# crockwell/rel_pose

Hardware: AMD Instinct MI355X
Metric: image-pairs/sec fwd+bwd @384x384, 1/2/4/8 MI355X; R,t err vs ref (higher is better)
Workload: dtype f32; 1 GPU; train.py step (ViTEss fwd + geodesic loss + bwd + grad all-reduce + clip + Adam), synthetic 384x384 pairs; scope=full, pairs_per_gpu=64, global_batch_pairs=64, parallelism=dp1, finite=True, gemm_operand_precision=exact fp32 MFMA, launch=eager

## Files before the change

__graft_entry__.py:

```python
import os
import subprocess
import sys

ROOT = os.path.dirname(os.path.abspath(__file__))
if ROOT not in sys.path:
    sys.path.insert(0, ROOT)


def build():
    import torch
    from rel_pose_amd import _build
    force = os.environ.get("RP_FORCE_BUILD", "" if torch.cuda.is_available() else "1") == "1"
    _build.build(force=force, verbose=True)
    from rel_pose_amd import _lib
    lib = _lib.load()
    assert lib.rp_abi_version() == _lib.ABI_VERSION and lib.rp_target_arch() == b"gfx950"
    assert lib.rp_abi_export_count() == _lib.ABI_EXPORTS == len(_lib.EXPORTS)
    assert _lib.load_readout().rp_readout_abi_version() == _lib.READOUT_ABI_VERSION
    assert _lib.load_eightpoint().rp_eightpoint_abi_version() == _lib.EIGHTPOINT_ABI_VERSION
    assert _lib.load_refine().rp_refine_abi_version() == _lib.REFINE_ABI_VERSION
    assert _lib.load_consensus().rp_consensus_abi_version() == _lib.CONSENSUS_ABI_VERSION
    assert _lib.load_submatch().rp_submatch_abi_version() == _lib.SUBMATCH_ABI_VERSION
    assert _lib.load_fivepoint().rp_fivepoint_abi_version() == _lib.FIVEPOINT_ABI_VERSION
    assert _lib.load_homography().rp_homography_abi_version() == _lib.HOMOGRAPHY_ABI_VERSION
    assert _lib.load_triangulate().rp_triangulate_abi_version() == _lib.TRIANGULATE_ABI_VERSION
    assert _lib.load_conv5x5().rp_conv5x5_abi_version() == _lib.CONV5X5_ABI_VERSION
    assert _lib.load_guided().rp_guided_abi_version() == _lib.GUIDED_ABI_VERSION
    assert _lib.load_rotation().rp_rotation_abi_version() == _lib.ROTATION_ABI_VERSION
    assert _lib.load_select().rp_select_abi_version() == _lib.SELECT_ABI_VERSION
    assert _lib.load_covariance().rp_covariance_abi_version() == _lib.COVARIANCE_ABI_VERSION
    assert _lib.load_resection().rp_resection_abi_version() == _lib.RESECTION_ABI_VERSION
    import rel_pose_amd.model
    import oracle.relpose_oracle
    print("build ok:", _lib.lib_path(), _build.READOUT_LIB, _build.EIGHTPOINT_LIB, _build.REFINE_LIB, _build.CONSENSUS_LIB, _build.SUBMATCH_LIB,
          _build.FIVEPOINT_LIB, _build.HOMOGRAPHY_LIB, _build.TRIANGULATE_LIB, _build.CONV5X5_LIB, _build.GUIDED_LIB, _build.ROTATION_LIB, _build.SELECT_LIB,
          _build.COVARIANCE_LIB, _build.RESECTION_LIB)


def smoke():
    import types

    import torch

    from oracle import relpose_oracle as O
    from rel_pose_amd import _lib
    from rel_pose_amd.model import ViTEss
    assert torch.cuda.is_available(), "smoke() needs cuda:0"
    _lib.load()
    torch.cuda.set_device(0)
    args = types.SimpleNamespace(noess="", pool_size=60, fc_hidden_size=512, fusion_transformer=True,
                                 transformer_depth=6, cross_features=False, use_single_softmax=False,
                                 no_pos_encoding=False, l1_pos_encoding=False)
    shapes = dict(O.vit_param_shapes())
    shapes.update(O.cnn_param_shapes())
    sd32, sd64 = O.make_state(shapes, torch.float32), O.make_state(shapes, torch.float64)
    model = ViTEss(args)
    model.load_state_dict(sd32)
    model = model.cuda().train()
    tok = O.synthetic_tokens(2)
    Gs = torch.tensor([0, 0, 0, 0, 0, 0, 1.0]).repeat(1, 2, 1)
    intr = torch.tensor([[30.0, 26.0, 12.0, 11.0]]).repeat(1, 2, 1)
    fmap = tok.permute(0, 2, 1).contiguous().view(2, 192, 24, 24).cuda().requires_grad_(True)
    out = model.forward_tokens(fmap, Gs.cuda(), intr.cuda())
    out[:, 1].square().sum().backward()
    t64 = tok.double().requires_grad_(True)
    ref = O.vit_ess_from_tokens(sd64, t64, Gs.double(), intr.double())
    ref[:, 1].square().sum().backward()
    t_err, q_err, ang = O.pose_errors(out.detach().cpu(), ref.detach())
    g_err = O.rel_err(fmap.grad.view(2, 192, 576).permute(0, 2, 1).cpu(), t64.grad)
    print("smoke: t_err=%.2e q_err=%.2e angle=%.2e rad, token-grad rel err=%.2e" % (t_err, q_err, ang, g_err))
    assert max(t_err, q_err) < 1e-4 and g_err < 2e-5
    print("smoke ok (HIP path vs CPU oracle)")


if __name__ == "__main__":
    build()
    if len(sys.argv) > 1 and sys.argv[1] == "smoke":
        smoke()
```

rel_pose_amd/_build.py:

```python
import os
import subprocess
import sys

HERE = os.path.dirname(os.path.abspath(__file__))
CSRC = os.path.join(HERE, "csrc")
LIB = os.path.join(HERE, "librelpose_hip.so")
SOURCES = ["gemm.hip", "gemm_dma.hip", "rowwise.hip", "attention.hip", "attention_bf16.hip", "dw192_bf16.hip", "dw192_f32.hip", "dw192_split3.hip", "dx_lnbwd_bf16.hip", "emm.hip", "emm_bf16.hip", "batchnorm.hip", "se3loss.hip", "geom.hip", "augment.hip", "mlp_fused.hip", "linear_rows.hip", "conv_stem.hip", "conv_stem_bf16.hip", "conv_stem_wgrad_bf16.hip", "conv_stem_wgrad_f32.hip", "conv3x3_bf16.hip", "conv3x3_wgrad_bf16.hip", "conv3x3_wgrad_f32.hip", "conv3x3_f32.hip", "conv3x3_c128_f32.hip"]
READOUT_CSRC = os.path.join(HERE, "csrc_readout")
READOUT_LIB = os.path.join(HERE, "librelpose_readout.so")
READOUT_SOURCES = ["emm_readout.hip"]
EIGHTPOINT_CSRC = os.path.join(HERE, "csrc_eightpoint")
EIGHTPOINT_LIB = os.path.join(HERE, "librelpose_eightpoint.so")
EIGHTPOINT_SOURCES = ["eight_point.hip"]
REFINE_CSRC = os.path.join(HERE, "csrc_refine")
REFINE_LIB = os.path.join(HERE, "librelpose_refine.so")
REFINE_SOURCES = ["refine_pose.hip"]
CONSENSUS_CSRC = os.path.join(HERE, "csrc_consensus")
CONSENSUS_LIB = os.path.join(HERE, "librelpose_consensus.so")
CONSENSUS_SOURCES = ["consensus.hip"]
SUBMATCH_CSRC = os.path.join(HERE, "csrc_submatch")
SUBMATCH_LIB = os.path.join(HERE, "librelpose_submatch.so")
SUBMATCH_SOURCES = ["submatch.hip"]
FIVEPOINT_CSRC = os.path.join(HERE, "csrc_fivepoint")
FIVEPOINT_LIB = os.path.join(HERE, "librelpose_fivepoint.so")
FIVEPOINT_SOURCES = ["five_point.hip"]
HOMOGRAPHY_CSRC = os.path.join(HERE, "csrc_homography")
HOMOGRAPHY_LIB = os.path.join(HERE, "librelpose_homography.so")
HOMOGRAPHY_SOURCES = ["homography.hip"]
TRIANGULATE_CSRC = os.path.join(HERE, "csrc_triangulate")
TRIANGULATE_LIB = os.path.join(HERE, "librelpose_triangulate.so")
TRIANGULATE_SOURCES = ["triangulate.hip"]
CONV5X5_CSRC = os.path.join(HERE, "csrc_conv5x5")
CONV5X5_LIB = os.path.join(HERE, "librelpose_conv5x5.so")
CONV5X5_SOURCES = ["conv5x5_dgrad_f32.hip"]
GUIDED_CSRC = os.path.join(HERE, "csrc_guided")
GUIDED_LIB = os.path.join(HERE, "librelpose_guided.so")
GUIDED_SOURCES = ["emm_guided.hip"]
ROTATION_CSRC = os.path.join(HERE, "csrc_rotation")
ROTATION_LIB = os.path.join(HERE, "librelpose_rotation.so")
ROTATION_SOURCES = ["rotation.hip"]
SELECT_CSRC = os.path.join(HERE, "csrc_select")
SELECT_LIB = os.path.join(HERE, "librelpose_select.so")
SELECT_SOURCES = ["select.hip"]
COVARIANCE_CSRC = os.path.join(HERE, "csrc_covariance")
COVARIANCE_LIB = os.path.join(HERE, "librelpose_covariance.so")
COVARIANCE_SOURCES = ["covariance.hip"]
RESECTION_CSRC = os.path.join(HERE, "csrc_resection")
RESECTION_LIB = os.path.join(HERE, "librelpose_resection.so")
RESECTION_SOURCES = ["resection.hip"]
ARCH = "gfx950"


def _hipcc():
    for c in (os.environ.get("HIPCC"), "/opt/rocm/bin/hipcc"):
        if c and os.path.exists(c):
            return c
    return "hipcc"


def _stale(lib, csrc, sources, headers):
    if not os.path.exists(lib):
        return True
    t = os.path.getmtime(lib)
    return any(os.path.getmtime(d) > t for d in [os.path.join(csrc, s) for s in sources] + headers)


def needs_build():
    return _stale(LIB, CSRC, SOURCES, _headers())


def readout_needs_build():
    return _stale(READOUT_LIB, READOUT_CSRC, READOUT_SOURCES, _readout_headers())


def eightpoint_needs_build():
    return _stale(EIGHTPOINT_LIB, EIGHTPOINT_CSRC, EIGHTPOINT_SOURCES, _eightpoint_headers())


def refine_needs_build():
    return _stale(REFINE_LIB, REFINE_CSRC, REFINE_SOURCES, _refine_headers())


def consensus_needs_build():
    return _stale(CONSENSUS_LIB, CONSENSUS_CSRC, CONSENSUS_SOURCES, _consensus_headers())


def submatch_needs_build():
    return _stale(SUBMATCH_LIB, SUBMATCH_CSRC, SUBMATCH_SOURCES, _submatch_headers())


def fivepoint_needs_build():
    return _stale(FIVEPOINT_LIB, FIVEPOINT_CSRC, FIVEPOINT_SOURCES, _fivepoint_headers())


def homography_needs_build():
    return _stale(HOMOGRAPHY_LIB, HOMOGRAPHY_CSRC, HOMOGRAPHY_SOURCES, _homography_headers())


def triangulate_needs_build():
    return _stale(TRIANGULATE_LIB, TRIANGULATE_CSRC, TRIANGULATE_SOURCES, _triangulate_headers())


def conv5x5_needs_build():
    return _stale(CONV5X5_LIB, CONV5X5_CSRC, CONV5X5_SOURCES, _conv5x5_headers())


def guided_needs_build():
    return _stale(GUIDED_LIB, GUIDED_CSRC, GUIDED_SOURCES, _guided_headers())


def rotation_needs_build():
    return _stale(ROTATION_LIB, ROTATION_CSRC, ROTATION_SOURCES, _rotation_headers())


def select_needs_build():
    return _stale(SELECT_LIB, SELECT_CSRC, SELECT_SOURCES, _select_headers())


def covariance_needs_build():
    return _stale(COVARIANCE_LIB, COVARIANCE_CSRC, COVARIANCE_SOURCES, _covariance_headers())


def resection_needs_build():
    return _stale(RESECTION_LIB, RESECTION_CSRC, RESECTION_SOURCES, _resection_headers())


def build(force=False, verbose=True):
    import fcntl
    with open(os.path.join(HERE, ".build.lock"), "w") as lock:
        fcntl.flock(lock, fcntl.LOCK_EX)
        try:
            if force or needs_build():
                _build_locked(verbose, force, LIB, CSRC, SOURCES, _headers())
            if force or readout_needs_build():
                _build_locked(verbose, force, READOUT_LIB, READOUT_CSRC, READOUT_SOURCES, _readout_headers())
            if force or eightpoint_needs_build():
                _build_locked(verbose, force, EIGHTPOINT_LIB, EIGHTPOINT_CSRC, EIGHTPOINT_SOURCES, _eightpoint_headers())
            if force or refine_needs_build():
                _build_locked(verbose, force, REFINE_LIB, REFINE_CSRC, REFINE_SOURCES, _refine_headers())
            if force or consensus_needs_build():
                _build_locked(verbose, force, CONSENSUS_LIB, CONSENSUS_CSRC, CONSENSUS_SOURCES, _consensus_headers())
            if force or submatch_needs_build():
                _build_locked(verbose, force, SUBMATCH_LIB, SUBMATCH_CSRC, SUBMATCH_SOURCES, _submatch_headers())
            if force or fivepoint_needs_build():
                _build_locked(verbose, force, FIVEPOINT_LIB, FIVEPOINT_CSRC, FIVEPOINT_SOURCES, _fivepoint_headers())
            if force or homography_needs_build():
                _build_locked(verbose, force, HOMOGRAPHY_LIB, HOMOGRAPHY_CSRC, HOMOGRAPHY_SOURCES, _homography_headers())
            if force or triangulate_needs_build():
                _build_locked(verbose, force, TRIANGULATE_LIB, TRIANGULATE_CSRC, TRIANGULATE_SOURCES, _triangulate_headers())
            if force or conv5x5_needs_build():
                _build_locked(verbose, force, CONV5X5_LIB, CONV5X5_CSRC, CONV5X5_SOURCES, _conv5x5_headers())
            if force or guided_needs_build():
                _build_locked(verbose, force, GUIDED_LIB, GUIDED_CSRC, GUIDED_SOURCES, _guided_headers())
            if force or rotation_needs_build():
                _build_locked(verbose, force, ROTATION_LIB, ROTATION_CSRC, ROTATION_SOURCES, _rotation_headers())
            if force or select_needs_build():
                _build_locked(verbose, force, SELECT_LIB, SELECT_CSRC, SELECT_SOURCES, _select_headers())
            if force or covariance_needs_build():
                _build_locked(verbose, force, COVARIANCE_LIB, COVARIANCE_CSRC, COVARIANCE_SOURCES, _covariance_headers())
            if force or resection_needs_build():
                _build_locked(verbose, force, RESECTION_LIB, RESECTION_CSRC, RESECTION_SOURCES, _resection_headers())
            return LIB
        finally:
            fcntl.flock(lock, fcntl.LOCK_UN)


def _headers():
    return [os.path.join(CSRC, h) for h in sorted(os.listdir(CSRC)) if h.endswith(".h")] + \
           [os.path.join(os.path.dirname(HERE), "include", "relpose_hip.h")]


def _readout_headers():
    return _headers() + [os.path.join(os.path.dirname(HERE), "include", "relpose_readout.h")]


def _eightpoint_headers():
    return _headers() + [os.path.join(os.path.dirname(HERE), "include", "relpose_eightpoint.h")]


def _refine_headers():
    return _headers() + [os.path.join(os.path.dirname(HERE), "include", "relpose_refine.h")]


def _consensus_headers():
    return _headers() + [os.path.join(os.path.dirname(HERE), "include", "relpose_consensus.h")]


def _submatch_headers():
    return _headers() + [os.path.join(os.path.dirname(HERE), "include", "relpose_submatch.h")]


def _fivepoint_headers():
    return _headers() + [os.path.join(os.path.dirname(HERE), "include", "relpose_fivepoint.h")]


def _homography_headers():
    return _headers() + [os.path.join(os.path.dirname(HERE), "include", "relpose_homography.h")]


def _triangulate_headers():
    return _headers() + [os.path.join(os.path.dirname(HERE), "include", "relpose_triangulate.h")]


def _conv5x5_headers():
    return _headers() + [os.path.join(os.path.dirname(HERE), "include", "relpose_conv5x5.h")]


def _guided_headers():
    return _headers() + [os.path.join(os.path.dirname(HERE), "include", "relpose_guided.h")]


def _rotation_headers():
    return _headers() + [os.path.join(os.path.dirname(HERE), "include", "relpose_rotation.h")]


def _select_headers():
    return _headers() + [os.path.join(os.path.dirname(HERE), "include", "relpose_select.h")]


def _covariance_headers():
    return _headers() + [os.path.join(COVARIANCE_CSRC, "sym5.h"), os.path.join(os.path.dirname(HERE), "include", "relpose_covariance.h")]


def _resection_headers():
    return _headers() + [os.path.join(os.path.dirname(HERE), "include", "relpose_resection.h")]


def _build_locked(verbose, force, lib, csrc, sources, headers):
    cc = _hipcc()
    objs = []
    procs = []
    hdr_t = max(os.path.getmtime(h) for h in headers)
    for s in sources:
        o = os.path.join(csrc, s.replace(".hip", ".o"))
        objs.append(o)
        if not force and os.path.exists(o) and os.path.getmtime(o) > max(hdr_t, os.path.getmtime(os.path.join(csrc, s))):
            continue
        cmd = [cc, "--offload-arch=" + ARCH, "-O3", "-std=c++17", "-fPIC", "-c", os.path.join(csrc, s), "-o", o]
        if verbose:
            print(" ".join(cmd), flush=True)
        procs.append((s, subprocess.Popen(cmd, stdout=subprocess.PIPE, stderr=subprocess.STDOUT)))
    for s, p in procs:
        out, _ = p.communicate()
        if p.returncode != 0:
            sys.stderr.write(out.decode())
            raise RuntimeError("hipcc failed on " + s)
    tmp = lib + ".tmp.%d" % os.getpid()
    cmd = [cc, "--offload-arch=" + ARCH, "-shared", "-fPIC", "-o", tmp] + objs
    if verbose:
        print(" ".join(cmd), flush=True)
    subprocess.check_call(cmd)
    os.replace(tmp, lib)
    return lib


if __name__ == "__main__":
    build(force="--force" in sys.argv)
```

rel_pose_amd/_lib.py:

```python
import ctypes
import keyword
import os
import re
from ctypes import POINTER, Structure, c_char_p, c_float, c_int, c_longlong, c_size_t, c_void_p

import torch

from . import _build

_LIB = None
HEADER = os.path.join(os.path.dirname(os.path.dirname(os.path.abspath(__file__))), "include", "relpose_hip.h")

_SCALARS = {"int": c_int, "float": c_float, "long long": c_longlong, "size_t": c_size_t}
_POINTEES = ("void", "float", "double", "int", "unsigned char")
_DEFINE = re.compile(r"#\s*define\s+(RP_\w+)\s+(-?\d+|\(-?\d+\))")
_DECL = re.compile(r"(const\s+)?(unsigned\s+char|long\s+long|\w+)\s*(\*?)\s*([A-Za-z_]\w*(?:\s*,\s*[A-Za-z_]\w*)*)?")
_ITEM = re.compile(r"\s*(?:typedef\s+struct\s+(\w+)\s*\{([^{}]*);\s*\}\s*(\w+)\s*;"
                   r"|([\w\s*]+?)\b(rp_\w+)\s*\(([^()]*)\)\s*;"
                   r'|extern\s+"C"\s*\{|\})')


def _declaration(text, structs, header="relpose_hip.h"):
    m = _DECL.fullmatch(text.strip())
    if not m:
# ... 136 lines not shown

_CONV5X5_LIB = None
CONV5X5_HEADER = os.path.join(os.path.dirname(HEADER), "relpose_conv5x5.h")
with open(CONV5X5_HEADER) as _f:
    _CONV5X5_CONSTS, _, _CONV5X5_PROTOTYPES, _CONV5X5_STATUS = _header_contract(_f.read(), "relpose_conv5x5.h")
CONV5X5_ABI_VERSION = _CONV5X5_CONSTS["RP_CONV5X5_ABI_VERSION"]
CONV5X5_EXPORTS = tuple(_CONV5X5_PROTOTYPES)


_GUIDED_LIB = None
GUIDED_HEADER = os.path.join(os.path.dirname(HEADER), "relpose_guided.h")
with open(GUIDED_HEADER) as _f:
    _GUIDED_CONSTS, _, _GUIDED_PROTOTYPES, _GUIDED_STATUS = _header_contract(_f.read(), "relpose_guided.h")
GUIDED_ABI_VERSION = _GUIDED_CONSTS["RP_GUIDED_ABI_VERSION"]
GUIDED_EXPORTS = tuple(_GUIDED_PROTOTYPES)


_ROTATION_LIB = None
ROTATION_HEADER = os.path.join(os.path.dirname(HEADER), "relpose_rotation.h")
with open(ROTATION_HEADER) as _f:
    _ROTATION_CONSTS, _, _ROTATION_PROTOTYPES, _ROTATION_STATUS = _header_contract(_f.read(), "relpose_rotation.h")
ROTATION_ABI_VERSION = _ROTATION_CONSTS["RP_ROTATION_ABI_VERSION"]
ROTATION_MAX_P, ROTATION_MAX_M, ROTATION_MAX_ITERS = (_ROTATION_CONSTS[k] for k in ("RP_ROTATION_MAX_P", "RP_ROTATION_MAX_M", "RP_ROTATION_MAX_ITERS"))
ROTATION_EXPORTS = tuple(_ROTATION_PROTOTYPES)


_SELECT_LIB = None
SELECT_HEADER = os.path.join(os.path.dirname(HEADER), "relpose_select.h")
with open(SELECT_HEADER) as _f:
    _SELECT_CONSTS, _, _SELECT_PROTOTYPES, _SELECT_STATUS = _header_contract(_f.read(), "relpose_select.h")
SELECT_ABI_VERSION = _SELECT_CONSTS["RP_SELECT_ABI_VERSION"]
SELECT_MAX_P, SELECT_MAX_C = _SELECT_CONSTS["RP_SELECT_MAX_P"], _SELECT_CONSTS["RP_SELECT_MAX_C"]
SELECT_EXPORTS = tuple(_SELECT_PROTOTYPES)


_COVARIANCE_LIB = None
COVARIANCE_HEADER = os.path.join(os.path.dirname(HEADER), "relpose_covariance.h")
with open(COVARIANCE_HEADER) as _f:
    _COVARIANCE_CONSTS, _, _COVARIANCE_PROTOTYPES, _COVARIANCE_STATUS = _header_contract(_f.read(), "relpose_covariance.h")
COVARIANCE_ABI_VERSION = _COVARIANCE_CONSTS["RP_COVARIANCE_ABI_VERSION"]
COVARIANCE_MAX_P, COVARIANCE_SWEEPS = _COVARIANCE_CONSTS["RP_COVARIANCE_MAX_P"], _COVARIANCE_CONSTS["RP_COVARIANCE_SWEEPS"]
COVARIANCE_EXPORTS = tuple(_COVARIANCE_PROTOTYPES)


_RESECTION_LIB = None
RESECTION_HEADER = os.path.join(os.path.dirname(HEADER), "relpose_resection.h")
with open(RESECTION_HEADER) as _f:
    _RESECTION_CONSTS, _, _RESECTION_PROTOTYPES, _RESECTION_STATUS = _header_contract(_f.read(), "relpose_resection.h")
RESECTION_ABI_VERSION = _RESECTION_CONSTS["RP_RESECTION_ABI_VERSION"]
RESECTION_MAX_P, RESECTION_MAX_M, RESECTION_MAX_ITERS = (_RESECTION_CONSTS[k] for k in ("RP_RESECTION_MAX_P", "RP_RESECTION_MAX_M", "RP_RESECTION_MAX_ITERS"))
RESECTION_EXPORTS = tuple(_RESECTION_PROTOTYPES)


def lib_path():
    return _build.LIB


def load():
    global _LIB
    if _LIB is not None:
        return _LIB
    path = _build.LIB
    if _build.needs_build():
        _build.build(verbose=False)
    try:
        lib = ctypes.CDLL(path)
    except OSError as e:
        raise RuntimeError("rel_pose_amd: cannot load HIP extension %s (%s); there is no CPU fallback" % (path, e))
    lib.rp_abi_version.restype = c_int
    if lib.rp_abi_version() != ABI_VERSION:
        raise RuntimeError("rel_pose_amd: %s has ABI version %d, this package binds version %d -- rebuild with "
                           "`python -m rel_pose_amd._build --force`" % (path, lib.rp_abi_version(), ABI_VERSION))
    if len(EXPORTS) != ABI_EXPORTS:
        raise RuntimeError("rel_pose_amd: include/relpose_hip.h declares %d entry points (RP_ABI_EXPORTS = %d)" % (len(EXPORTS), ABI_EXPORTS))
    lib.rp_abi_export_count.restype = c_int
    if lib.rp_abi_export_count() != ABI_EXPORTS:
        raise RuntimeError("rel_pose_amd: %s was compiled with %d entry points, the header declares %d -- rebuild"
                           % (path, lib.rp_abi_export_count(), ABI_EXPORTS))
    for name, (res, args) in _PROTOTYPES.items():
        fn = getattr(lib, name)
        fn.restype = res
        fn.argtypes = args
        if name in _STATUS:
            fn.errcheck = _raise_on_status
    _LIB = lib
    return lib


def load_readout():
    global _READOUT_LIB
    if _READOUT_LIB is not None:
        return _READOUT_LIB
    path = _build.READOUT_LIB
    if _build.readout_needs_build():
        _build.build(verbose=False)
    try:
        lib = ctypes.CDLL(path)
    except OSError as e:
        raise RuntimeError("rel_pose_amd: cannot load HIP extension %s (%s); there is no CPU fallback" % (path, e))
    lib.rp_readout_abi_version.restype = c_int
    if lib.rp_readout_abi_version() != READOUT_ABI_VERSION:
        raise RuntimeError("rel_pose_amd: %s has ABI version %d, this package binds version %d -- rebuild with "
                           "`python -m rel_pose_amd._build --force`" % (path, lib.rp_readout_abi_version(), READOUT_ABI_VERSION))
    for name, (res, args) in _READOUT_PROTOTYPES.items():
        fn = getattr(lib, name)
        fn.restype = res
# ... 279 lines not shown
    return lib


def load_covariance():
    global _COVARIANCE_LIB
    if _COVARIANCE_LIB is not None:
        return _COVARIANCE_LIB
    path = _build.COVARIANCE_LIB
    if _build.covariance_needs_build():
        _build.build(verbose=False)
    try:
        lib = ctypes.CDLL(path)
    except OSError as e:
        raise RuntimeError("rel_pose_amd: cannot load HIP extension %s (%s); there is no CPU fallback" % (path, e))
    lib.rp_covariance_abi_version.restype = c_int
    if lib.rp_covariance_abi_version() != COVARIANCE_ABI_VERSION:
        raise RuntimeError("rel_pose_amd: %s has ABI version %d, this package binds version %d -- rebuild with "
                           "`python -m rel_pose_amd._build --force`" % (path, lib.rp_covariance_abi_version(), COVARIANCE_ABI_VERSION))
    for name, (res, args) in _COVARIANCE_PROTOTYPES.items():
        fn = getattr(lib, name)
        fn.restype = res
        fn.argtypes = args
        if name in _COVARIANCE_STATUS:
            fn.errcheck = _raise_on_status
    _COVARIANCE_LIB = lib
    return lib


def load_resection():
    global _RESECTION_LIB
    if _RESECTION_LIB is not None:
        return _RESECTION_LIB
    path = _build.RESECTION_LIB
    if _build.resection_needs_build():
        _build.build(verbose=False)
    try:
        lib = ctypes.CDLL(path)
    except OSError as e:
        raise RuntimeError("rel_pose_amd: cannot load HIP extension %s (%s); there is no CPU fallback" % (path, e))
    lib.rp_resection_abi_version.restype = c_int
    if lib.rp_resection_abi_version() != RESECTION_ABI_VERSION:
        raise RuntimeError("rel_pose_amd: %s has ABI version %d, this package binds version %d -- rebuild with "
                           "`python -m rel_pose_amd._build --force`" % (path, lib.rp_resection_abi_version(), RESECTION_ABI_VERSION))
    for name, (res, args) in _RESECTION_PROTOTYPES.items():
        fn = getattr(lib, name)
        fn.restype = res
        fn.argtypes = args
        if name in _RESECTION_STATUS:
            fn.errcheck = _raise_on_status
    _RESECTION_LIB = lib
    return lib


def _raise_on_status(rc, func, args):
    check(rc, func.__name__)
    return rc


def check(rc, what):
    if rc != 0:
        if rc < 0:
            raise RuntimeError("rel_pose_amd: %s failed: %s (RP error %d)" % (what, RP_ERRORS.get(rc, "?"), rc))
        raise RuntimeError("rel_pose_amd: %s failed: hipError %d" % (what, rc))
```

rel_pose_amd/ops.py:

```python
import ctypes
import itertools
import math
import os
import threading

import torch

from . import _lib

N_TOK = 576
DIM = 192
HEADS = 3
LN_EPS = 1e-6
XW = 96
GW = 224
NWG = 6


def _chk(*ts):
    for t in ts:
        if t is None:
            continue
        if not (t.is_cuda and t.dtype == torch.float32 and t.is_contiguous()):
            raise RuntimeError("rel_pose_amd ops need contiguous fp32 GPU tensors (no CPU fallback exists); got "
# ... 1789 lines not shown
                dw = torch.ops.aten.convolution_backward(dy, x, w, None, [1, 1], [1, 1], [1, 1], False, [0, 0], 1, [False, True, False])[1]
        return dx, dw, None, None, None


CONV3X3_C128_F32 = os.environ.get("RP_CONV3X3_C128_F32", "1") != "0"
CONV_F32_STATS = os.environ.get("RP_CONV_F32_STATS", "1") != "0"
CONV3X3_C128_F32_MIN_N = int(os.environ.get("RP_CONV3X3_C128_F32_MIN_N", "56"))


def conv3x3_c128_f32(x_nhwc, w_ohwi, bias=None, input_gradient=False, want_stats=False):
    lib = _lib.load()
    if not (x_nhwc.is_cuda and x_nhwc.is_contiguous() and x_nhwc.dtype == torch.float32 and tuple(x_nhwc.shape[1:]) == (28, 28, 128)):
        raise RuntimeError("conv3x3_c128_f32: contiguous fp32 [N,28,28,128] GPU tensor expected")
    CO = w_ohwi.shape[0]
    if not (w_ohwi.is_cuda and w_ohwi.is_contiguous() and w_ohwi.dtype == torch.float32 and tuple(w_ohwi.shape[1:]) == (3, 3, 128)
            and CO in (128, 192)):
        raise RuntimeError("conv3x3_c128_f32: contiguous fp32 [128 | 192,3,3,128] GPU filter expected")
    if input_gradient and (CO != 128 or bias is not None):
        raise RuntimeError("conv3x3_c128_f32: the input gradient needs the square 128 -> 128 filter and takes no bias")
    if bias is not None and not (bias.is_cuda and bias.is_contiguous() and bias.dtype == torch.float32 and tuple(bias.shape) == (CO,)):
        raise RuntimeError("conv3x3_c128_f32: contiguous fp32 [CO] GPU bias expected")
    N = x_nhwc.shape[0]
    y = torch.empty(N, 28, 28, CO, device=x_nhwc.device, dtype=torch.float32)
    stats = (torch.empty(lib.rp_conv3x3_c128_f32_blocks(N, CO) // (CO // 64), 2, CO, device=x_nhwc.device, dtype=torch.float64)
             if want_stats else None)
    with timed("conv3x3_c128_f32", 2.0 * N * 28 * 28 * 128 * CO * 9, 4.0 * N * 28 * 28 * (128 + CO)):
        lib.rp_conv3x3_c128_f32(_p(x_nhwc), _p(w_ohwi), _p(bias), _p(y), _p(stats), N, 28, 28, CO, 1 if input_gradient else 0,
                                _st())
    return (y, stats) if want_stats else y


class Conv3x3C128F32Fn(_Fn):

    @staticmethod
    def forward(ctx, x, w, bias, want_stats=False):
        ctx.save_for_backward(x, w)
        ctx.has_bias = bias is not None
        if want_stats and CONV_F32_STATS:
            y, stats = conv3x3_c128_f32(_nhwc(x), _nhwc(w), bias, want_stats=True)
            ctx.mark_non_differentiable(stats)
            return y.permute(0, 3, 1, 2), stats
        y = conv3x3_c128_f32(_nhwc(x), _nhwc(w), bias).permute(0, 3, 1, 2)
        return (y, None) if want_stats else y

    @staticmethod
    def backward(ctx, dy, *_):
        x, w = ctx.saved_tensors
        dx = dw = db = None
        dy = dy.contiguous(memory_format=torch.channels_last)
        CO = w.shape[0]
        own_dx = ctx.needs_input_grad[0] and CO == 128
        if own_dx:
            dx = conv3x3_c128_f32(_nhwc(dy), _nhwc(w), input_gradient=True).permute(0, 3, 1, 2)
        mask = [bool(ctx.needs_input_grad[0]) and not own_dx, bool(ctx.needs_input_grad[1]), ctx.has_bias and bool(ctx.needs_input_grad[2])]
        if any(mask):
            g = torch.ops.aten.convolution_backward(dy, x, w, [CO] if ctx.has_bias else None, [1, 1], [1, 1], [1, 1], False, [0, 0], 1, mask)
            dx = g[0] if mask[0] else dx
            dw = g[1] if mask[1] else None
            db = g[2] if mask[2] else None
        return dx, dw, db, None


def conv3x3_c128_f32_ok(m, x):
    return (CONV3X3_C128_F32 and CNN_PRECISION == 0 and x.is_cuda and x.dtype == torch.float32 and tuple(m.weight.shape[1:]) == (128, 3, 3)
            and m.weight.shape[0] in (128, 192) and m.stride == (1, 1) and m.padding == (1, 1) and m.dilation == (1, 1) and m.groups == 1
            and getattr(m, "padding_mode", "zeros") == "zeros" and tuple(x.shape[1:]) == (128, 28, 28) and x.shape[0] >= CONV3X3_C128_F32_MIN_N)


CONV5X5_DGRAD_F32 = os.environ.get("RP_CONV5X5_DGRAD_F32", "1") != "0"
CONV5X5_DGRAD_F32_MIN_N = int(os.environ.get("RP_CONV5X5_DGRAD_F32_MIN_N", "112"))
CONV5X5_DGRAD_IMAGES = 128


def conv5x5_dgrad_f32(dy_nhwc, w_ohwi, res_nhwc=None):
    lib = _lib.load_conv5x5()
    if not (dy_nhwc.is_cuda and dy_nhwc.is_contiguous() and dy_nhwc.dtype == torch.float32 and dy_nhwc.dim() == 4
            and tuple(dy_nhwc.shape[1:]) == (24, 24, 192) and dy_nhwc.shape[0] >= 1):
        raise RuntimeError("conv5x5_dgrad_f32: contiguous fp32 [N,24,24,192] GPU tensor expected")
    CI = w_ohwi.shape[-1]
    if not (w_ohwi.is_cuda and w_ohwi.is_contiguous() and w_ohwi.dtype == torch.float32 and tuple(w_ohwi.shape[:3]) == (192, 5, 5)
            and CI in (128, 192)):
        raise RuntimeError("conv5x5_dgrad_f32: contiguous fp32 [192,5,5,128 | 192] GPU filter expected")
    N = dy_nhwc.shape[0]
    if res_nhwc is not None and not (res_nhwc.is_cuda and res_nhwc.is_contiguous() and res_nhwc.dtype == torch.float32
                                     and tuple(res_nhwc.shape) == (N, 28, 28, CI)):
        raise RuntimeError("conv5x5_dgrad_f32: contiguous fp32 [N,28,28,CI] GPU residual expected")
    dx = torch.empty(N, 28, 28, CI, device=dy_nhwc.device, dtype=torch.float32)
    lib.rp_conv5x5_dgrad_f32(_p(dy_nhwc), _p(w_ohwi), _p(dx), N, CI, _p(res_nhwc), _st())
    return dx


class Conv5x5ValidF32Fn(_Fn):

    @staticmethod
    def forward(ctx, x, w, bias):
        ctx.save_for_backward(x, w)
        ctx.has_bias = bias is not None
        return torch.nn.functional.conv2d(x, w, bias)

    @staticmethod
    def backward(ctx, dy):
        x, w = ctx.saved_tensors
        dx = dw = db = None
        dy = dy.contiguous(memory_format=torch.channels_last)
        if ctx.needs_input_grad[0]:
            dx = conv5x5_dgrad_f32(_nhwc(dy), _nhwc(w)).permute(0, 3, 1, 2)
        mask = [False, bool(ctx.needs_input_grad[1]), ctx.has_bias and bool(ctx.needs_input_grad[2])]
        if any(mask):
            g = torch.ops.aten.convolution_backward(dy, x, w, [192] if ctx.has_bias else None, [1, 1], [0, 0], [1, 1], False, [0, 0], 1, mask)
            dw = g[1] if mask[1] else None
            db = g[2] if mask[2] else None
        return dx, dw, db


def conv5x5_dgrad_f32_ok(m, x):
    n = x.shape[0]
    return (CONV5X5_DGRAD_F32 and CNN_PRECISION == 0 and x.is_cuda and x.dtype == torch.float32 and torch.is_grad_enabled()
            and x.requires_grad and tuple(m.kernel_size) == (5, 5) and m.stride == (1, 1) and m.padding == (0, 0) and m.dilation == (1, 1)
            and m.groups == 1 and m.weight.shape[0] == 192 and tuple(x.shape[1:]) in ((192, 28, 28), (128, 28, 28))
            and tuple(m.weight.shape[1:]) == (x.shape[1], 5, 5) and n >= CONV5X5_DGRAD_F32_MIN_N
            and (n - 1) % CONV5X5_DGRAD_IMAGES + 1 >= CONV5X5_DGRAD_F32_MIN_N)


def conv3x3_wgrad_f32_ok(m, x):
    return (CONV3X3_WGRAD_F32 and CNN_PRECISION == 0 and x.is_cuda and x.dtype == torch.float32 and torch.is_grad_enabled()
            and m.weight.requires_grad and tuple(m.weight.shape) == (64, 64, 3, 3) and m.bias is None and m.stride == (1, 1)
            and m.padding == (1, 1) and m.dilation == (1, 1) and m.groups == 1 and tuple(x.shape[1:]) == (64, 56, 56)
            and x.shape[0] >= CONV3X3_WGRAD_F32_MIN_N)


def conv3x3_f32_ok(m, x):
    return (CONV3X3_F32 and CNN_PRECISION == 0 and x.is_cuda and x.dtype == torch.float32 and tuple(m.weight.shape) == (64, 64, 3, 3)
            and m.bias is None and m.stride == (1, 1) and m.padding == (1, 1) and m.dilation == (1, 1) and m.groups == 1
            and tuple(x.shape[1:]) == (64, 56, 56) and x.shape[0] >= CONV3X3_F32_MIN_N)


def conv3x3_own_ok(m, x):
    return (CONV3X3_OWN and CNN_PRECISION == 1 and x.is_cuda and tuple(m.weight.shape) == (64, 64, 3, 3) and m.bias is None
            and m.stride == (1, 1) and m.padding == (1, 1) and m.dilation == (1, 1) and m.groups == 1 and tuple(x.shape[1:]) == (64, 56, 56))


def conv2d(m, x, want_stats=False):
    if want_stats:
        if conv3x3_own_ok(m, x) and getattr(m, "_rp_bf16", None) is not None:
            xb = x if x.dtype == torch.bfloat16 else x.to(torch.bfloat16)
            return Conv3x3C64Fn.apply(xb, m._rp_bf16[0], True)
        if CNN_PRECISION == 0 and x.is_cuda and torch.is_grad_enabled():
            bn_src = getattr(x, "_rp_bn", None) if CONV_F32_BN_BWD else None
            if conv3x3_f32_ok(m, x):
                return Conv3x3C64F32Fn.apply(x, m.weight, True, False, bn_src)
            if conv3x3_c128_f32_ok(m, x):
                return Conv3x3C128F32Fn.apply(x, m.weight, m.bias, True)
        return conv2d(m, x), None
    if CNN_PRECISION == 0 or not x.is_cuda:
        if conv3x3_wgrad_f32_ok(m, x) or conv3x3_f32_ok(m, x):
            return Conv3x3C64F32Fn.apply(x, m.weight, False, False, None)
        if conv3x3_c128_f32_ok(m, x):
            return Conv3x3C128F32Fn.apply(x, m.weight, m.bias, False)
        if conv5x5_dgrad_f32_ok(m, x):
            return Conv5x5ValidF32Fn.apply(x, m.weight, m.bias)
        return m(x)
    bf = torch.bfloat16
    ready = getattr(m, "_rp_bf16", None)
    if ready is not None and conv3x3_own_ok(m, x):
        return Conv3x3C64Fn.apply(x if x.dtype == bf else x.to(bf), ready[0], False)
    if ready is not None:
        xb = x if x.dtype == bf else x.to(bf)
        if (m.stride == (1, 1) and m.dilation == (1, 1) and m.groups == 1 and m.kernel_size[0] == m.kernel_size[1]
                and m.kernel_size[0] >= CONV_BWD_AS_FWD_MIN_K):
            return ConvBf16Fn.apply(xb, ready[0], ready[1], m.padding)
        return torch.nn.functional.conv2d(xb, ready[0], ready[1], m.stride, m.padding, m.dilation, m.groups)
    return torch.nn.functional.conv2d(x if x.dtype == bf else x.to(bf), m.weight.to(bf), None if m.bias is None else m.bias.to(bf),
                                      m.stride, m.padding, m.dilation, m.groups)

# ... 367 lines not shown
```

Measured before the change: 2000 image-pairs/sec.

## Add split-K MFMA fp32 weight-gradient kernel for 3x3 and 5x5 convs at 28x28

Adds a new HIP library with a weight-gradient kernel for the 28x28 3x3 (pad 1) and 5x5 (valid) convolutions. It stages input rows in an LDS ring buffer and output-gradient rows in a double buffer via global-to-LDS DMA, overlapped with fp32 MFMA accumulation over taps. Work is split over image-row ranges into a workspace, and a second kernel reduces the partials. The backward passes of those conv autograd functions call it instead of aten convolution_backward for dw. This adds a workspace allocation and an extra reduction launch, and it changes the summation order relative to the library kernel.

```diff
diff --git a/__graft_entry__.py b/__graft_entry__.py
--- a/__graft_entry__.py
+++ b/__graft_entry__.py
@@ -30,11 +30,12 @@
     assert _lib.load_select().rp_select_abi_version() == _lib.SELECT_ABI_VERSION
     assert _lib.load_covariance().rp_covariance_abi_version() == _lib.COVARIANCE_ABI_VERSION
     assert _lib.load_resection().rp_resection_abi_version() == _lib.RESECTION_ABI_VERSION
+    assert _lib.load_convwgrad().rp_convwgrad_abi_version() == _lib.CONVWGRAD_ABI_VERSION
     import rel_pose_amd.model
     import oracle.relpose_oracle
     print("build ok:", _lib.lib_path(), _build.READOUT_LIB, _build.EIGHTPOINT_LIB, _build.REFINE_LIB, _build.CONSENSUS_LIB, _build.SUBMATCH_LIB,
           _build.FIVEPOINT_LIB, _build.HOMOGRAPHY_LIB, _build.TRIANGULATE_LIB, _build.CONV5X5_LIB, _build.GUIDED_LIB, _build.ROTATION_LIB, _build.SELECT_LIB,
-          _build.COVARIANCE_LIB, _build.RESECTION_LIB)
+          _build.COVARIANCE_LIB, _build.RESECTION_LIB, _build.CONVWGRAD_SO)
 
 
 def smoke():
diff --git a/include/relpose_convwgrad.h b/include/relpose_convwgrad.h
--- /dev/null
+++ b/include/relpose_convwgrad.h
@@ -0,0 +1,23 @@
+#ifndef RELPOSE_CONVWGRAD_H
+#define RELPOSE_CONVWGRAD_H
+
+#include "relpose_hip.h"
+
+#ifdef __cplusplus
+extern "C" {
+#endif
+
+#define RP_CONVWGRAD_ABI_VERSION 1
+int rp_convwgrad_abi_version(void);
+
+int rp_conv_wgrad_f32_runs(int CI, int CO, int KS);
+int rp_conv_wgrad_f32_blocks(int CI, int CO, int KS);
+size_t rp_conv_wgrad_f32_workspace_bytes(int CI, int CO, int KS);
+
+int rp_conv_wgrad_f32(const float* x, const float* dy, float* dw, void* workspace, size_t workspace_bytes, int N, int CI, int CO, int KS,
+                      void* stream);
+
+#ifdef __cplusplus
+}
+#endif
+#endif
diff --git a/rel_pose_amd/_build.py b/rel_pose_amd/_build.py
--- a/rel_pose_amd/_build.py
+++ b/rel_pose_amd/_build.py
@@ -48,6 +48,9 @@
 RESECTION_CSRC = os.path.join(HERE, "csrc_resection")
 RESECTION_LIB = os.path.join(HERE, "librelpose_resection.so")
 RESECTION_SOURCES = ["resection.hip"]
+CONVWGRAD_CSRC = os.path.join(HERE, "csrc_convwgrad")
+CONVWGRAD_SO = os.path.join(HERE, "librelpose_convwgrad.so")
+CONVWGRAD_SOURCES = ["conv_wgrad_f32.hip"]
 ARCH = "gfx950"
 
 
@@ -123,6 +126,10 @@
 
 def resection_needs_build():
     return _stale(RESECTION_LIB, RESECTION_CSRC, RESECTION_SOURCES, _resection_headers())
+
+
+def convwgrad_needs_build():
+    return _stale(CONVWGRAD_SO, CONVWGRAD_CSRC, CONVWGRAD_SOURCES, _convwgrad_headers())
 
 
 def build(force=False, verbose=True):
@@ -160,6 +167,8 @@
                 _build_locked(verbose, force, COVARIANCE_LIB, COVARIANCE_CSRC, COVARIANCE_SOURCES, _covariance_headers())
             if force or resection_needs_build():
                 _build_locked(verbose, force, RESECTION_LIB, RESECTION_CSRC, RESECTION_SOURCES, _resection_headers())
+            if force or convwgrad_needs_build():
+                _build_locked(verbose, force, CONVWGRAD_SO, CONVWGRAD_CSRC, CONVWGRAD_SOURCES, _convwgrad_headers())
             return LIB
         finally:
             fcntl.flock(lock, fcntl.LOCK_UN)
@@ -224,6 +233,10 @@
 
 def _resection_headers():
     return _headers() + [os.path.join(os.path.dirname(HERE), "include", "relpose_resection.h")]
+
+
+def _convwgrad_headers():
+    return _headers() + [os.path.join(os.path.dirname(HERE), "include", "relpose_convwgrad.h")]
 
 
 def _build_locked(verbose, force, lib, csrc, sources, headers):
diff --git a/rel_pose_amd/_lib.py b/rel_pose_amd/_lib.py
--- a/rel_pose_amd/_lib.py
+++ b/rel_pose_amd/_lib.py
@@ -212,6 +212,14 @@
 RESECTION_EXPORTS = tuple(_RESECTION_PROTOTYPES)
 
 
+_CONVWGRAD_LIB = None
+CONVWGRAD_HEADER = os.path.join(os.path.dirname(HEADER), "relpose_convwgrad.h")
+with open(CONVWGRAD_HEADER) as _f:
+    _CONVWGRAD_CONSTS, _, _CONVWGRAD_PROTOTYPES, _CONVWGRAD_STATUS = _header_contract(_f.read(), "relpose_convwgrad.h")
+CONVWGRAD_ABI_VERSION = _CONVWGRAD_CONSTS["RP_CONVWGRAD_ABI_VERSION"]
+CONVWGRAD_EXPORTS = tuple(_CONVWGRAD_PROTOTYPES)
+
+
 def lib_path():
     return _build.LIB
 
@@ -597,6 +605,31 @@
     return lib
 
 
+def load_convwgrad():
+    global _CONVWGRAD_LIB
+    if _CONVWGRAD_LIB is not None:
+        return _CONVWGRAD_LIB
+    path = _build.CONVWGRAD_SO
+    if _build.convwgrad_needs_build():
+        _build.build(verbose=False)
+    try:
+        lib = ctypes.CDLL(path)
+    except OSError as e:
+        raise RuntimeError("rel_pose_amd: cannot load HIP extension %s (%s); there is no CPU fallback" % (path, e))
+    lib.rp_convwgrad_abi_version.restype = c_int
+    if lib.rp_convwgrad_abi_version() != CONVWGRAD_ABI_VERSION:
+        raise RuntimeError("rel_pose_amd: %s has ABI version %d, this package binds version %d -- rebuild with "
+                           "`python -m rel_pose_amd._build --force`" % (path, lib.rp_convwgrad_abi_version(), CONVWGRAD_ABI_VERSION))
+    for name, (res, args) in _CONVWGRAD_PROTOTYPES.items():
+        fn = getattr(lib, name)
+        fn.restype = res
+        fn.argtypes = args
+        if name in _CONVWGRAD_STATUS:
+            fn.errcheck = _raise_on_status
+    _CONVWGRAD_LIB = lib
+    return lib
+
+
 def _raise_on_status(rc, func, args):
     check(rc, func.__name__)
     return rc
diff --git a/rel_pose_amd/csrc_convwgrad/conv_wgrad_f32.hip b/rel_pose_amd/csrc_convwgrad/conv_wgrad_f32.hip
--- /dev/null
+++ b/rel_pose_amd/csrc_convwgrad/conv_wgrad_f32.hip
@@ -0,0 +1,212 @@
+#include "../csrc/common.h"
+#include "../../include/relpose_convwgrad.h"
+
+namespace {
+
+constexpr int IH = 28, IW = 28;
+constexpr int CB = 64;
+constexpr int NPX = IW / 4;
+
+template <int KS> struct Geo {
+  static constexpr int PAD = KS == 3 ? 1 : 0;
+  static constexpr int OH = IH + 2 * PAD - KS + 1;
+  static constexpr int T = KS * KS;
+  static constexpr int NGRP = KS == 3 ? 1 : 2;
+  static constexpr int NT0 = (T + NGRP - 1) / NGRP;
+  static constexpr int NR = 3;
+  static constexpr int XSLOT = (IW + 2 * PAD) * CB;
+  static constexpr int RING = KS == 3 ? 8 : 16;
+  static constexpr int NSLOT = RING + (PAD ? 1 : 0);
+  static constexpr int YROW = OH * CB;
+  static constexpr int NPY = OH / 4;
+  static constexpr int KSTEPS = OH / 2;
+  static constexpr int MAXP = (KS == 3 ? 1 : NR) * NPX + NPY;
+  static_assert(MAXP <= 4 * KSTEPS, "one DMA piece per wave and k-step");
+};
+
+struct Wg {
+  const float* x;
+  const float* dy;
+  float* ws;
+  int N, CI, CO, S;
+};
+
+template <int KS, int R0> RP_DEV int row_lo(int t) {
+  constexpr int OH = Geo<KS>::OH;
+  if constexpr (KS == 3) return t - (t % OH > 0 ? 1 : 0);
+  else return (t / OH) * IH + t % OH + R0;
+}
+template <int KS, int R0> RP_DEV int row_hi(int t, int nrows) {
+  if constexpr (KS == 3) return min(t + 1, nrows - 1);
+  else return row_lo<KS, R0>(t) + Geo<KS>::NR - 1;
+}
+
+template <int NT> RP_DEV void wait_operands(float& a, float (&b)[NT]) {
+  asm volatile("s_waitcnt lgkmcnt(0)" : "+v"(a));
+#pragma unroll
+  for (int i = 0; i < NT; ++i) asm volatile("" : "+v"(b[i]));
+}
+
+template <int KS, int TAP0, int NT>
+RP_DEV void wgrad_body(const Wg& p, float* Xr, float* Ys, int chan, int j) {
+  using G = Geo<KS>;
+  constexpr int PAD = G::PAD, OH = G::OH, T = G::T, XSLOT = G::XSLOT, YROW = G::YROW, NPY = G::NPY, KSTEPS = G::KSTEPS, NR = G::NR;
+  constexpr int R0 = TAP0 / KS;
+  static_assert((TAP0 + NT - 1) / KS - R0 + 1 == NR && NT <= 16, "a group spans NR filter rows and fits the AGPRs");
+  const int tid = threadIdx.x, lane = tid & 63, wave = __builtin_amdgcn_readfirstlane(tid >> 6), l31 = lane & 31, hi = lane >> 5;
+  const int coh = wave >> 1, cih = wave & 1;
+  const int cbs = p.CI / CB, cob = chan / cbs, cib = chan - cob * cbs;
+  const int nrows = p.N * IH, ntiles = p.N * OH;
+  const int t0 = (int)((long long)ntiles * j / p.S), t1 = (int)((long long)ntiles * (j + 1) / p.S);
+
+  if constexpr (PAD) {
+    for (int i = tid; i < G::RING * 2 * CB; i += 256) Xr[(i >> 7) * XSLOT + ((i >> 6) & 1) * (IW + 1) * CB + (i & 63)] = 0.f;
+    for (int i = tid; i < XSLOT; i += 256) Xr[G::RING * XSLOT + i] = 0.f;
+  }
+
+  f32x16 acc[NT];
+#pragma unroll
+  for (int t = 0; t < NT; ++t) acc[t] = zero16();
+
+  const unsigned xs0 = lds_byte_addr(Xr), ys0 = lds_byte_addr(Ys);
+  const unsigned xl = (unsigned)(((lane >> 4) * p.CI + (lane & 15) * 4) * 4), yl = (unsigned)(((lane >> 4) * p.CO + (lane & 15) * 4) * 4);
+  const unsigned xq = (unsigned)(16 * p.CI), yq = (unsigned)(16 * p.CO);
+  const float* xb = p.x + cib * CB;
+  const float* yb = p.dy + cob * CB;
+  auto dma_x = [&](int row, int q) {
+    glds16(uniform_ptr(xb + (long long)row * (IW * p.CI)), q * xq + xl,
+           __builtin_amdgcn_readfirstlane(xs0 + (row & (G::RING - 1)) * (XSLOT * 4) + PAD * (CB * 4) + q * 1024));
+  };
+  auto dma_y = [&](int row, int q) {
+    glds16(uniform_ptr(yb + (long long)row * (OH * p.CO)), q * yq + yl, __builtin_amdgcn_readfirstlane(ys0 + (row & 1) * (YROW * 4) + q * 1024));
+  };
+  auto issue = [&](int q, int xrow0, int nx, int yrow) {
+    if (q < nx) {
+      const int r = q / NPX;
+      dma_x(xrow0 + r, q - r * NPX);
+    } else if (q < nx + NPY) dma_y(yrow, q - nx);
+  };
+  if (t0 < t1) {
+    const int lo = row_lo<KS, R0>(t0), nx = (row_hi<KS, R0>(t0, nrows) - lo + 1) * NPX;
+    for (int q = wave; q < nx + NPY; q += 4) issue(q, lo, nx, t0);
+  }
+  asm volatile("s_waitcnt vmcnt(0) lgkmcnt(0)" ::: "memory");
+  __builtin_amdgcn_s_barrier();
+
+  const unsigned xoff = (32 * cih + l31) * 4 + hi * (CB * 4), yoff = (32 * coh + l31) * 4 + hi * (CB * 4);
+  for (int t = t0; t < t1; ++t) {
+    const int n = t / OH, y = t - n * OH;
+    const int xn = max(row_hi<KS, R0>(t, nrows) + 1, row_lo<KS, R0>(t + 1));
+    const int nx = t + 1 < t1 ? (row_hi<KS, R0>(t + 1, nrows) - xn + 1) * NPX : 0;
+    const int np = t + 1 < t1 ? nx + NPY : 0;
+    const unsigned ya = ys0 + (t & 1) * (YROW * 4) + yoff;
+    unsigned xa[NR];
+#pragma unroll
+    for (int r = 0; r < NR; ++r) {
+      const int yy = y + R0 + r - PAD, g = n * IH + yy;
+      const int slot = (PAD && (yy < 0 || yy >= IH)) ? G::RING : (g & (G::RING - 1));
+      xa[r] = xs0 + slot * (XSLOT * 4) + xoff;
+    }
+    float a, bq[NT];
+    a = lds_rd32<0>(ya);
+    static_for<NT>([&](auto i) { bq[i] = lds_rd32<((TAP0 + i) % KS) * CB * 4>(xa[(TAP0 + i) / KS - R0]); });
+    static_for<KSTEPS>([&](auto kc) {
+      constexpr int k = kc;
+      wait_operands(a, bq);
+      float an = 0.f, bn[NT] = {};
+      if constexpr (k + 1 < KSTEPS) {
+        constexpr int o = 2 * (k + 1) * CB * 4;
+        an = lds_rd32<o>(ya);
+        static_for<NT>([&](auto i) { bn[i] = lds_rd32<o + ((TAP0 + i) % KS) * CB * 4>(xa[(TAP0 + i) / KS - R0]); });
+      }
+      if constexpr (4 * k < G::MAXP) {
+        if (wave + 4 * k < np) issue(wave + 4 * k, xn, nx, t + 1);
+      }
+      __builtin_amdgcn_sched_barrier(0);
+#pragma unroll
+      for (int i = 0; i < NT; ++i) acc[i] = mfma32(a, bq[i], acc[i]);
+      if constexpr (k + 1 < KSTEPS) {
+        a = an;
+#pragma unroll
+        for (int i = 0; i < NT; ++i) bq[i] = bn[i];
+      }
+    });
+    asm volatile("s_waitcnt vmcnt(0) lgkmcnt(0)" ::: "memory");
+    __builtin_amdgcn_s_barrier();
+  }
+  float* o = p.ws + ((long long)chan * p.S + j) * (CB * T * CB) + (32 * coh) * (T * CB) + TAP0 * CB + 32 * cih + l31;
+#pragma unroll
+  for (int i = 0; i < NT; ++i)
+#pragma unroll
+    for (int r = 0; r < 16; ++r) o[acc_row(r, hi) * (T * CB) + i * CB] = acc[i][r];
+}
+
+template <int KS>
+__global__ __launch_bounds__(256, 1) void conv_wgrad_f32_kernel(Wg p) {
+  using G = Geo<KS>;
+  __shared__ __attribute__((aligned(16))) float Xr[G::NSLOT * G::XSLOT];
+  __shared__ __attribute__((aligned(16))) float Ys[2 * G::YROW];
+  const int units = (p.CO / CB) * (p.CI / CB) * G::NGRP, per = (units * p.S + 7) / 8;
+  const int b = blockIdx.x, L = (b & 7) * per + (b >> 3);
+  const int j = L / units, unit = L - j * units;
+  if (j >= p.S) return;
+  if constexpr (G::NGRP == 1) wgrad_body<KS, 0, G::T>(p, Xr, Ys, unit, j);
+  else if (unit & 1) wgrad_body<KS, G::NT0, G::T - G::NT0>(p, Xr, Ys, unit >> 1, j);
+  else wgrad_body<KS, 0, G::NT0>(p, Xr, Ys, unit >> 1, j);
+}
+
+__global__ __launch_bounds__(256) void conv_wgrad_f32_reduce_kernel(const float* __restrict__ ws, float* __restrict__ dw, int S, int T, int CI) {
+  __shared__ float4 part[4][64];
+  const int o = threadIdx.x & 63, sl = threadIdx.x >> 6;
+  const int e = (blockIdx.x * 64 + o) * 4;
+  const int ci = e % CI, tap = (e / CI) % T, co = e / (CI * T);
+  const int chan = (co / CB) * (CI / CB) + ci / CB;
+  const float* src = ws + (long long)chan * S * (CB * T * CB) + (co % CB) * (T * CB) + tap * CB + ci % CB;
+  const int k0 = S * sl / 4, k1 = S * (sl + 1) / 4;
+  float4 s = make_float4(0.f, 0.f, 0.f, 0.f);
+  for (int k = k0; k < k1; ++k) {
+    const float4 v = ld4(src + (long long)k * (CB * T * CB));
+    s.x += v.x; s.y += v.y; s.z += v.z; s.w += v.w;
+  }
+  part[sl][o] = s;
+  __syncthreads();
+  if (sl == 0) {
+    const float4 p0 = part[0][o], p1 = part[1][o], p2 = part[2][o], p3 = part[3][o];
+    st4(dw + e, make_float4(((p0.x + p1.x) + p2.x) + p3.x, ((p0.y + p1.y) + p2.y) + p3.y, ((p0.z + p1.z) + p2.z) + p3.z,
+                            ((p0.w + p1.w) + p2.w) + p3.w));
+  }
+}
+
+bool supported(int CI, int CO, int KS) {
+  return (KS == 3 && CI == 128 && (CO == 128 || CO == 192)) || (KS == 5 && CO == 192 && (CI == 128 || CI == 192));
+}
+int units(int CI, int CO, int KS) { return (CI / CB) * (CO / CB) * (KS == 3 ? 1 : 2); }
+int runs(int CI, int CO, int KS) { return 256 / units(CI, CO, KS); }
+
+}
+
+extern "C" int rp_convwgrad_abi_version(void) { return RP_CONVWGRAD_ABI_VERSION; }
+
+extern "C" int rp_conv_wgrad_f32_runs(int CI, int CO, int KS) { return supported(CI, CO, KS) ? runs(CI, CO, KS) : 0; }
+extern "C" int rp_conv_wgrad_f32_blocks(int CI, int CO, int KS) { return supported(CI, CO, KS) ? units(CI, CO, KS) * runs(CI, CO, KS) : 0; }
+extern "C" size_t rp_conv_wgrad_f32_workspace_bytes(int CI, int CO, int KS) {
+  return supported(CI, CO, KS) ? (size_t)(CI / CB) * (CO / CB) * runs(CI, CO, KS) * CB * KS * KS * CB * sizeof(float) : 0;
+}
+
+extern "C" int rp_conv_wgrad_f32(const float* x, const float* dy, float* dw, void* workspace, size_t workspace_bytes, int N, int CI, int CO,
+                                 int KS, void* stream) {
+  if (!x || !dy || !dw || !workspace || N < 1) return RP_EBADSHAPE;
+  if (!supported(CI, CO, KS)) return RP_EUNSUPPORTED;
+  if (((uintptr_t)x | (uintptr_t)dy | (uintptr_t)dw | (uintptr_t)workspace) & 15) return RP_EALIGN;
+  if (workspace_bytes < rp_conv_wgrad_f32_workspace_bytes(CI, CO, KS)) return RP_EWORKSPACE;
+  const int S = runs(CI, CO, KS);
+  Wg p{x, dy, (float*)workspace, N, CI, CO, S};
+  const dim3 grid((units(CI, CO, KS) * S + 7) / 8 * 8);
+  hipStream_t st = (hipStream_t)stream;
+  if (KS == 3) hipLaunchKernelGGL(conv_wgrad_f32_kernel<3>, grid, dim3(256), 0, st, p);
+  else hipLaunchKernelGGL(conv_wgrad_f32_kernel<5>, grid, dim3(256), 0, st, p);
+  RP_CHECK_LAUNCH();
+  hipLaunchKernelGGL(conv_wgrad_f32_reduce_kernel, dim3(CO * KS * KS * CI / 256), dim3(256), 0, st, (const float*)workspace, dw, S, KS * KS, CI);
+  RP_CHECK_LAUNCH();
+  return RP_OK;
+}
diff --git a/rel_pose_amd/ops.py b/rel_pose_amd/ops.py
--- a/rel_pose_amd/ops.py
+++ b/rel_pose_amd/ops.py
@@ -1865,11 +1865,15 @@
         own_dx = ctx.needs_input_grad[0] and CO == 128
         if own_dx:
             dx = conv3x3_c128_f32(_nhwc(dy), _nhwc(w), input_gradient=True).permute(0, 3, 1, 2)
-        mask = [bool(ctx.needs_input_grad[0]) and not own_dx, bool(ctx.needs_input_grad[1]), ctx.has_bias and bool(ctx.needs_input_grad[2])]
+        own_dw = bool(ctx.needs_input_grad[1]) and conv_wgrad_f32_ok(x, w, (1, 1), (1, 1))
+        if own_dw:
+            dw = conv_wgrad_f32(_nhwc(x), _nhwc(dy), 3).permute(0, 3, 1, 2)
+        mask = [bool(ctx.needs_input_grad[0]) and not own_dx, bool(ctx.needs_input_grad[1]) and not own_dw,
+                ctx.has_bias and bool(ctx.needs_input_grad[2])]
         if any(mask):
             g = torch.ops.aten.convolution_backward(dy, x, w, [CO] if ctx.has_bias else None, [1, 1], [1, 1], [1, 1], False, [0, 0], 1, mask)
             dx = g[0] if mask[0] else dx
-            dw = g[1] if mask[1] else None
+            dw = g[1] if mask[1] else dw
             db = g[2] if mask[2] else None
         return dx, dw, db, None
 
@@ -1918,10 +1922,13 @@
         dy = dy.contiguous(memory_format=torch.channels_last)
         if ctx.needs_input_grad[0]:
             dx = conv5x5_dgrad_f32(_nhwc(dy), _nhwc(w)).permute(0, 3, 1, 2)
-        mask = [False, bool(ctx.needs_input_grad[1]), ctx.has_bias and bool(ctx.needs_input_grad[2])]
+        own_dw = bool(ctx.needs_input_grad[1]) and conv_wgrad_f32_ok(x, w, (1, 1), (0, 0))
+        if own_dw:
+            dw = conv_wgrad_f32(_nhwc(x), _nhwc(dy), 5).permute(0, 3, 1, 2)
+        mask = [False, bool(ctx.needs_input_grad[1]) and not own_dw, ctx.has_bias and bool(ctx.needs_input_grad[2])]
         if any(mask):
             g = torch.ops.aten.convolution_backward(dy, x, w, [192] if ctx.has_bias else None, [1, 1], [0, 0], [1, 1], False, [0, 0], 1, mask)
-            dw = g[1] if mask[1] else None
+            dw = g[1] if mask[1] else dw
             db = g[2] if mask[2] else None
         return dx, dw, db
 
@@ -1933,6 +1940,43 @@
             and m.groups == 1 and m.weight.shape[0] == 192 and tuple(x.shape[1:]) in ((192, 28, 28), (128, 28, 28))
             and tuple(m.weight.shape[1:]) == (x.shape[1], 5, 5) and n >= CONV5X5_DGRAD_F32_MIN_N
             and (n - 1) % CONV5X5_DGRAD_IMAGES + 1 >= CONV5X5_DGRAD_F32_MIN_N)
+
+
+CONV_WGRAD_F32 = os.environ.get("RP_CONV_WGRAD_F32", "1") != "0"
+CONV_WGRAD_F32_MIN_N = int(os.environ.get("RP_CONV_WGRAD_F32_MIN_N", "64"))
+CONV_WGRAD_F32_GEOMETRIES = frozenset([(3, 128, 128), (3, 128, 192), (5, 192, 192)])
+_CONV_WGRAD_KINDS = frozenset([(3, 128, 128), (3, 128, 192), (5, 128, 192), (5, 192, 192)])
+
+
+def conv_wgrad_f32(x_nhwc, dy_nhwc, ks):
+    lib = _lib.load_convwgrad()
+    if not (x_nhwc.is_cuda and x_nhwc.is_contiguous() and x_nhwc.dtype == torch.float32 and x_nhwc.dim() == 4
+            and tuple(x_nhwc.shape[1:3]) == (28, 28) and x_nhwc.shape[0] >= 1):
+        raise RuntimeError("conv_wgrad_f32: contiguous fp32 [N,28,28,CI] GPU input expected")
+    N, CI = x_nhwc.shape[0], x_nhwc.shape[3]
+    if ks not in (3, 5):
+        raise RuntimeError("conv_wgrad_f32: ks is 3 (pad 1) or 5 (valid)")
+    oh = 28 if ks == 3 else 24
+    if not (dy_nhwc.is_cuda and dy_nhwc.is_contiguous() and dy_nhwc.dtype == torch.float32 and dy_nhwc.dim() == 4
+            and tuple(dy_nhwc.shape[:3]) == (N, oh, oh)):
+        raise RuntimeError("conv_wgrad_f32: contiguous fp32 [N,%d,%d,CO] GPU output gradient expected" % (oh, oh))
+    CO = dy_nhwc.shape[3]
+    if (ks, CI, CO) not in _CONV_WGRAD_KINDS:
+        raise RuntimeError("conv_wgrad_f32: (ks, CI, CO) is one of (3,128,128), (3,128,192), (5,128,192), (5,192,192)")
+    nb = lib.rp_conv_wgrad_f32_workspace_bytes(CI, CO, ks)
+    ws = _workspace(nb, x_nhwc.device)
+    dw = torch.empty(CO, ks, ks, CI, device=x_nhwc.device, dtype=torch.float32)
+    lib.rp_conv_wgrad_f32(_p(x_nhwc), _p(dy_nhwc), _p(dw), _p(ws), ws.numel() * 4, N, CI, CO, ks, _st())
+    return dw
+
+
+def conv_wgrad_f32_ok(x, w, stride=(1, 1), padding=(0, 0)):
+    if not (CONV_WGRAD_F32 and CNN_PRECISION == 0 and x.is_cuda and x.dtype == torch.float32 and w.dtype == torch.float32
+            and x.dim() == 4 and w.dim() == 4 and tuple(stride) == (1, 1) and x.shape[0] >= max(CONV_WGRAD_F32_MIN_N, 1)):
+        return False
+    ks = w.shape[2]
+    return (w.shape[3] == ks and tuple(padding) == ((1, 1) if ks == 3 else (0, 0)) and tuple(x.shape[2:]) == (28, 28)
+            and w.shape[1] == x.shape[1] and (ks, w.shape[1], w.shape[0]) in CONV_WGRAD_F32_GEOMETRIES)
 
 
 def conv3x3_wgrad_f32_ok(m, x):
```

Result: no change. 2006 image-pairs/sec (median of 6 runs) (+0.3%).
